# csiro-robotics/syropod_highlevel_controller

Hardware: AMD Instinct MI355X
Metric: control-cycles/sec (all legs IK-solved) (higher is better)
Workload: dtype f64

## Files before the change

### syropod_highlevel_controller_amd/csrc/shc_cycle_kernel.hpp

```cpp
#pragma once

#include "shc_cycle.hpp"
#include "shc_cycle_launch.hpp"

#include <hip/hip_runtime.h>

namespace shc {

#ifndef SHC_WAVES_PER_SIMD
#define SHC_WAVES_PER_SIMD 2
#endif
#ifndef SHC_ROT_WAVES_PER_SIMD
#define SHC_ROT_WAVES_PER_SIMD 1
#endif
#ifndef SHC_TERRAIN_WAVES_PER_SIMD
#define SHC_TERRAIN_WAVES_PER_SIMD 2
#endif

struct LegPlanes {
  double2 *base;
  int64_t ns;
  uint32_t slot;
  typedef double v2d __attribute__((ext_vector_type(2)));
  __device__ __forceinline__ double2 load(int plane) const { return (base + plane * ns)[slot]; }
// ... 343 lines not shown
    if (A.batch_mask & (1u << RG_IMU)) {
      const double *q = bound_array(A, 0, BND_IMUQ) + r * A.kstride[BND_IMUQ], *w = bound_array(A, 0, BND_IMUW) + r * A.kstride[BND_IMUW];
#pragma unroll
      for (int h = 0; h < NI; ++h) {
        const int idx = lane + 64 * h, field = idx / RPW, rr = idx - field * RPW;
        const int64_t rob = rob0 + rr;
        if (field < 7 && rob < st.n_robots) rob_imu[h] = field < 3 ? w[rob * 3 + field] : q[rob * 4 + (field - 3)];
      }
    }
  };
  const auto batch_rob_commit = [&]() {
    if (A.batch_mask & (1u << RG_VEL)) {
      const int field = lane / RPW, rr = lane - field * RPW;
      if (lane < 3 * RPW && wave * RPW + rr < st.n_robots) tile[(R::VIN + field) * RPW + rr] = rob_vel;
    }
    if (A.batch_mask & (1u << RG_IMU)) {
#pragma unroll
      for (int h = 0; h < NI; ++h) {
        const int idx = lane + 64 * h, field = idx / RPW, rr = idx - field * RPW;
        if (field < 7 && wave * RPW + rr < st.n_robots) tile[(R::GYRO + field) * RPW + rr] = rob_imu[h];
      }
      __builtin_amdgcn_fence(__ATOMIC_RELEASE, "wavefront");
      __builtin_amdgcn_wave_barrier();
      if (lane < RPW && wave * RPW + lane < st.n_robots) {
        const Quat qn = normalized(Quat{tile[(R::IMUQ + 0) * RPW + lane], tile[(R::IMUQ + 1) * RPW + lane], tile[(R::IMUQ + 2) * RPW + lane], tile[(R::IMUQ + 3) * RPW + lane]});
        tile[(R::IMUQ + 0) * RPW + lane] = qn.w, tile[(R::IMUQ + 1) * RPW + lane] = qn.x, tile[(R::IMUQ + 2) * RPW + lane] = qn.y, tile[(R::IMUQ + 3) * RPW + lane] = qn.z;
      }
    }
    __builtin_amdgcn_fence(__ATOMIC_RELEASE, "wavefront");
    __builtin_amdgcn_wave_barrier();
  };
  if constexpr (batch) batch_rob_issue(0);
  for (;;) {
    unsigned db = unsigned(gate), sp = unsigned(gate >> 32);
    if constexpr (batch) {
      if (c >= sp) break;
      h0 = u64(c) + 1, h1 = u64(A.batch_mask) | kResidentDirect;
      hdr_valid = true;
    }
    if (!batch && !(c < db && c < sp)) {
      if (c >= sp) break;
      asm volatile("s_waitcnt vmcnt(0)" ::: "memory");
      if (lane == 0) st_agent(A.progress + wave, u64(c));
      const u64 t0 = wall_clock64();
      for (;;) {
        __builtin_amdgcn_s_sleep(4);
        gate = uni64(ld_agent(&A.ctl->gate));
        db = unsigned(gate), sp = unsigned(gate >> 32);
        if (c >= sp || c < db) break;
        if (wall_clock64() - t0 > emergency_ticks) {
          held.fault = true;
          break;
        }
      }
      if (held.fault || c >= sp) break;
      hdr_valid = false;
    }
    if (!hdr_valid) {
      const u64 *hp = reinterpret_cast<const u64 *>(A.headers + (c & (kResidentHeaders - 1)));
      h0 = uni64(ld_agent(hp));
      h1 = uni64(ld_agent(hp + 1));
    }
    u64 gate_next_v = gate;
    if constexpr (!batch) gate_next_v = ld_agent(&A.ctl->gate);
    const bool next_valid = !batch && db > c + 1;
    u64 n0v = 0, n1v = 0;
    if (next_valid) {
      const u64 *hp = reinterpret_cast<const u64 *>(A.headers + ((c + 1) & (kResidentHeaders - 1)));
      n0v = ld_agent(hp);
      n1v = ld_agent(hp + 1);
    }
    const int64_t row = batch ? int64_t(c) : 0;
    if constexpr (batch) {
      held.seen |= A.batch_mask;
      if (A.batch_mask & (1u << RG_FORCE)) held.src_force = -2;
      if (A.batch_mask & (1u << RG_EFFORT)) held.src_effort = -2;
      batch_rob_commit();
      if (c + 1 < A.batch_cycles) batch_rob_issue(int64_t(c) + 1);
    } else {
      resident_take_inputs<64 / L, ROBOT_ALL, true>(A, c, h0, h1, wave, lane, tile, tile_i, dirty, held, st.n_robots, row);
    }
// ... 68 lines not shown
    const V3 f = in.force();
    planes[(FD::FORCE_IN / 2) * ns + slot] = double2{f.x, f.y};
    planes[(FD::FORCE_IN / 2 + 1) * ns + slot] = double2{f.z, 0.0};
  }
  if (held.src_effort != -1) {
    double ef[NJ];
    in.effort(ef);
#pragma unroll
    for (int p = 0; p < FD::NJE / 2; ++p) planes[(FD::EFFORT_IN / 2 + p) * ns + slot] = double2{ef[2 * p], 2 * p + 1 < NJ ? ef[2 * p + 1] : 0.0};
  }
}

template <int L, int NJ, unsigned F>
__device__ __forceinline__ void resident_epilogue(const ResidentArgs &A, const DevState &st, const uint32_t slot, const int lane, const bool live,
                                                  const double *tile, const int32_t *tile_i, double *gtile, int32_t *gtile_i, const ResidentHeld &held) {
  using R = RobotFields;
  using FD = Fields<NJ>;
  constexpr int RPW = 64 / L;
  const int64_t ns = st.n_slots;
  store_rob_fields<RPW, R::VIN, R::CORE_END>(tile, gtile, lane);
  if (held.seen & (1u << RG_IMU)) {
    store_rob_fields<RPW, R::GYRO, R::IMU_END>(tile, gtile, lane);
    store_rob_fields<RPW, R::IMUQ, R::IMUQ_END>(tile, gtile, lane);
  }
  if ((held.seen & (1u << RG_RESET)) && lane < RPW) gtile_i[R::I_RESET_MODE * RPW + lane] = tile_i[R::I_RESET_MODE * RPW + lane];
  if (live) carry_leg_inputs<L, NJ>(A, st, held, ns, slot, int(slot % 64) % L);
  if (lane == 0 && A.batch_cycles == 0) {
    if (held.fault) __hip_atomic_fetch_or(&A.ctl->fault, 1ull, __ATOMIC_RELAXED, __HIP_MEMORY_SCOPE_AGENT);
    __hip_atomic_fetch_add(&A.ctl->exited, 1ull, __ATOMIC_RELAXED, __HIP_MEMORY_SCOPE_AGENT);
  }
}

enum : int { PART_BOTH = 0, PART_GATE = 1, PART_DONE = 2 };
template <int PART>
__device__ __forceinline__ void resident_relay(const ResidentArgs &A) {
  const int lane = threadIdx.x & 63;
  const unsigned max_cycles = A.max_cycles;
  unsigned db = 0, sp = max_cycles, idle_stop = 0xffffffffu;
  u64 reason = RESIDENT_EXIT_MAX, last_reason = 0, last_gate = ~0ull, last_done = 0, iter = 0;
  u64 t_last = wall_clock64(), t_all_done = 0;
  for (;;) {
    const u64 now = wall_clock64();
    const u64 exited_v = ld_agent(&A.ctl->exited);
    const u64 gate_v = PART == PART_DONE ? ld_agent(&A.ctl->gate) : 0;
    const u64 done_v = PART != PART_DONE ? ld_agent(&A.ctl->pad[1]) : 0;
    u64 pv[8];
    if (PART != PART_GATE) {
#pragma unroll
      for (int j = 0; j < 8; ++j) pv[j] = j * 64 + lane < A.n_waves ? ld_agent(A.progress + j * 64 + lane) : ~0ull;
    }
    if (PART != PART_DONE) {
      const u64 hd_v = ld_sys(&A.host->doorbell), hs_v = ld_sys(&A.host->stop);
      const u64 rec_v = lane < 2 ? ld_sys(&A.host->records[size_t(db & (kResidentHeaders - 1)) * 2 + lane]) : 0;
      const u64 hd = uni64(hd_v), hs = uni64(hs_v);
      unsigned want_db = hd > max_cycles ? max_cycles : unsigned(hd);
      if (want_db < db) want_db = db;
      if (want_db == db && db < max_cycles) {
        const u64 tag = u64(db) + 1;
        const bool word_ok = lane == 0 ? rec_v == tag : (lane == 1 ? (rec_v >> 48) == (tag & 0xffffull) : true);
        if (__all(word_ok)) {
          const u64 w1 = uni64(__shfl(rec_v, 1, 64));
          if (lane == 0) {
            u64 *hp = reinterpret_cast<u64 *>(A.headers + (db & (kResidentHeaders - 1)));
            st_agent(hp + 1, (w1 & 0x7fffull) | u64(kResidentDirect) | (w1 & 0x30000ull));
            st_agent(hp, tag);
          }
          asm volatile("s_waitcnt vmcnt(0)" ::: "memory");
          want_db = db + 1;
        }
      }
      if (want_db != db || uni64(done_v) < u64(db)) t_last = now;
      else if (idle_stop == 0xffffffffu && now - t_last > A.idle_ticks) idle_stop = db;
      unsigned want_sp = max_cycles;
      u64 why = RESIDENT_EXIT_MAX;
      if (hs <= max_cycles) want_sp = unsigned(hs), why = RESIDENT_EXIT_STOP;
      if (idle_stop < want_sp) want_sp = idle_stop, why = RESIDENT_EXIT_IDLE;
      if (want_sp < db) want_sp = db;
      if (want_db > want_sp) want_db = want_sp;
      db = want_db, sp = want_sp, reason = why;
      if (reason != last_reason) {
        if (lane == 0) st_agent(&A.ctl->pad[0], reason);
        last_reason = reason;
      }
      const u64 gate = (u64(sp) << 32) | db;
      if (gate != last_gate) {
        if (lane == 0) st_agent(&A.ctl->gate, gate);
        last_gate = gate;
      }
    }
    const u64 exited = uni64(exited_v);
    bool leave = exited == u64(A.n_waves);
    if (PART != PART_GATE) {
      if (PART == PART_DONE) sp = unsigned(uni64(gate_v) >> 32);
      u64 m = ~0ull;
#pragma unroll
      for (int j = 0; j < 8; ++j) m = pv[j] < m ? pv[j] : m;
      for (int64_t base = 512; base < A.n_waves; base += 512) {
        u64 v[8];
#pragma unroll
        for (int j = 0; j < 8; ++j) {
          const int64_t w = base + j * 64 + lane;
          v[j] = w < A.n_waves ? ld_agent(A.progress + w) : ~0ull;
        }
#pragma unroll
        for (int j = 0; j < 8; ++j) m = v[j] < m ? v[j] : m;
      }
#pragma unroll
      for (int off = 32; off > 0; off >>= 1) {
        const u64 o = __shfl_xor(m, off, 64);
        m = o < m ? o : m;
      }
      m = uni64(m);
      if (m != last_done) {
        if (lane == 0) {
          st_sys(&A.host->done, m);
          st_agent(&A.ctl->pad[1], m);
        }
        last_done = m;
      }
      bool gave_up = false;
      if (!leave && m >= sp) {
        if (t_all_done == 0) t_all_done = now;
        else if (now - t_all_done > 5000 * A.ticks_per_ms) leave = gave_up = true;
      }
      if (leave) {
        const u64 fault = uni64(ld_agent(&A.ctl->fault));
        const u64 why = uni64(ld_agent(&A.ctl->pad[0]));
        if (lane == 0) {
          st_sys(&A.host->fault, fault);
          st_sys(&A.host->done, m);
          st_agent(&A.ctl->pad[1], m);
          asm volatile("s_waitcnt vmcnt(0)" ::: "memory");
          st_agent(&A.ctl->pad[2], 1ull);
          st_sys(&A.host->exited, (fault || gave_up) ? u64(RESIDENT_EXIT_FAULT) : why);
        }
      }
      if ((++iter & 1023) == 0 && lane == 0) st_sys(&A.host->heartbeat, iter);
    }
    if (leave) break;
    __builtin_amdgcn_s_sleep(1);
  }
}

template <int L, int NJ, unsigned F, bool RES, int HALF = ROLE_ALL, bool BATCH = false>
__device__ __forceinline__ void cycle_wave(const DevState &st, const SharedConsts<L, NJ> *gc, int n_cycles, unsigned rt_flags, const int64_t wave,
                                           const ResidentArgs *ra) {
  static_assert(HALF == ROLE_ALL || (!RES && (F & (F_DYN | F_TERRAIN | F_MLEGS | F_AUTO)) == 0), "half-step launches: feature-exact kernels without auto posing / terrain paths");
  using R = RobotFields;
  using FT = Feat<F>;
  constexpr int RPW = 64 / L;
  __shared__ SharedConsts<L, NJ> C;
  extern __shared__ double wave_lds[];
  constexpr int kWaveDoubles = R::COUNT * RPW + PK_COUNT * 64 + (R::I_COUNT * RPW + 1) / 2;
  SHC_TICK(0);
  const bool manual_live = (rt_flags & RT_MANUAL_LIVE) != 0;
  const bool touchdown_detection = (rt_flags & RT_TOUCHDOWN) != 0;
  const int lane = threadIdx.x & 63;
  const int wib = threadIdx.x >> 6;
  const int64_t rob0 = wave * RPW;
  const int64_t left = st.n_robots - rob0;
  const int robots_here = left < RPW ? (left < 0 ? 0 : int(left)) : RPW;
  int grp = lane / L;
  const int leg = lane - grp * L;
  const bool live = grp < robots_here;
  if (grp >= robots_here) grp = robots_here > 0 ? robots_here - 1 : 0;
// ... 430 lines not shown
#ifdef SHC_ABLATE
        if (!(P.debug_skip & 65536))
#endif
        if (POSE_SPLIT) publish_for_pose(c_front + 1, fb.plane_prev_changed);
        SHC_TICK(29);
        double *mb = &X.mailbox[pair][c_front & 1][0][lane];
        mb[0] = out.poser_tip.x, mb[64] = out.poser_tip.y, mb[128] = out.poser_tip.z;
        if constexpr (ODOM_WALKER) {
          if (FT::odom(P) && __any(fb.odom_run)) {
            if (fb.odom_run) {
              if constexpr (ODOM_REGS) odometry_advance(odom[0], odom[1], odom[2], odom[3], P, fb.odom_vel.x, fb.odom_vel.y, fb.odom_vel.z, &odom_cache);
              else odometry_step(rb, P, fb.odom_vel.x, fb.odom_vel.y, fb.odom_vel.z, &odom_cache);
            }
          }
        } else if (FT::odom(P)) {
          mb[192] = fb.odom_vel.x, mb[256] = fb.odom_vel.y, mb[320] = fb.odom_vel.z, mb[384] = fb.odom_run ? 1.0 : 0.0;
        }
        SHC_TICK(22);
      }
      SHC_TICK(23);
      if (kind == IT_EXIT) break;
      SHC_R2_ITER_END(0, 19, 20, 21, 2, 3, 4, 5, 6, 7, 16, 8, 17, 15, 29, 22, 23);
      if (kind == IT_REAL) ++c_front;
      prev_real = kind == IT_REAL;
      __syncthreads();
      ++k;
    }
  } else {
    for (;;) {
      SHC_R2_ITER_BEGIN();
      const int kind = __builtin_amdgcn_readfirstlane(int(X.ctrl[k & 3][0]));
      const u64 h0 = uni64(X.ctrl[k & 3][1]), h1 = uni64(X.ctrl[k & 3][2]);
      SHC_TICK(29);
      int nk = IT_EXIT;
      u64 nh0v = 0, nh1v = 0;
      if (leader && kind != IT_EXIT) {
        u64 gate;
        if (kind == IT_BUBBLE) {
          __builtin_amdgcn_s_sleep(2);
          gate = uni64(ld_agent(&A.ctl->gate));
        } else {
          gate = uni64(gate_pref);
        }
        const unsigned db = unsigned(gate), sp = unsigned(gate >> 32);
        const unsigned cn = c_front + (kind == IT_REAL ? 1u : 0u);
        nk = cn >= sp ? IT_EXIT : (cn < db ? IT_REAL : IT_BUBBLE);
        if (nk == IT_BUBBLE) {
          const u64 now = wall_clock64();
          if (bubble_since == 0) bubble_since = now;
          else if (now - bubble_since > emergency_ticks) nk = IT_EXIT, held.fault = true;
        } else {
          bubble_since = 0;
        }
        if (nk == IT_REAL) {
          const u64 *hp = reinterpret_cast<const u64 *>(A.headers + (cn & (kResidentHeaders - 1)));
          nh0v = ld_agent(hp);
          nh1v = ld_agent(hp + 1);
        }
        if (kind == IT_BUBBLE) gate_pref = gate;
        else gate_pref = ld_agent(&A.ctl->gate);
      }
      if (active) {
        SHC_TICK(24);
        if constexpr (POSE_SPLIT) if (kind == IT_REAL) {
          resident_take_inputs<RPW, ROBOT_POSE, false>(A, c_front, h0, h1, wave, lane, tile, tile_i, dirty, held, st.n_robots);
          SHC_TICK(30);
          double pose_c = -1.0;
#pragma unroll
          for (int j = 0; j < L; ++j) {
            const double cj = X.pose_c[pair][c_front & 1][g.base + j];
            pose_c = cj >= 0.0 ? cj : pose_c;
          }
          int lw[L] = {};
          const double *mb = &X.mailbox[pair][c_front & 1][0][lane];
          const V3 plane_prev{mb[7 * 64], mb[8 * 64], mb[9 * 64]}, pnorm_prev{mb[10 * 64], mb[11 * 64], mb[12 * 64]};
          int rword_unused = 0;
          Pose ap = pose_identity(), la = pose_identity();
#ifdef SHC_ABLATE
          if (!(P.debug_skip & 2048))
#endif
          (void)cycle_pose<L, NJ, F, true>(s, C, P, C.leg[leg], rb, g, leg, lw, rword_unused, 0, dirty, manual_live, ap, la, plane_prev, pnorm_prev, fb.uf.swing_c_count, 0,
                                           &owpp_cache, &pose_c);
          __builtin_amdgcn_fence(__ATOMIC_RELEASE, "workgroup");
          __builtin_amdgcn_wave_barrier();
          if (lane == 0) *const_cast<volatile unsigned *>(&X.pose_done[pair]) = c_front + 1;
        }
        SHC_TICK(25);
        if (prev_real) {
          resident_take_inputs<RPW, ROBOT_NONE, true>(A, c_back, prev_h0, prev_h1, wave, lane, tile, tile_i, dirty, held, st.n_robots);
          if (held.src_force != in_src_force || held.src_effort != in_src_effort) {
            in_at = leg_inputs_in_force<L, NJ>(A, st.legd, held.src_force, held.src_effort, ns, slot, wave * RPW + grp, leg);
            in_src_force = held.src_force, in_src_effort = held.src_effort;
          }
          LegInRing<NJ> in = in_at;
          if (FT::tipf(P)) in.prefetch_effort();
          SHC_TICK(31);
// ... 8 lines not shown
              }
            }
          }
          out.adm_delta = V3{0, 0, 0};
          if (FT::adm(P)) cycle_admittance<NJ>(s, out, P, in);
          s.word = 0;
          SHC_TICK(26);
          cycle_back<L, NJ, F>(s, out, C, leg, st.legd, ns, slot, nullptr, in, fb);
          SHC_TICK(27);
          asm volatile("s_waitcnt vmcnt(0)" ::: "memory");
          if (lane == 0) st_agent(A.progress + wave, u64(c_back));
          SHC_TICK(13);
          {
            typedef unsigned v4u __attribute__((ext_vector_type(4)));
            double flat[2 * NJ];
#pragma unroll
            for (int i = 0; i < NJ; ++i) flat[FD::Q + i] = s.q[i], flat[FD::QD + i] = s.qd[i];
            const unsigned soff = oslot * out_slot_bytes;
#ifdef SHC_ABLATE
            if (!(P.debug_skip & 4096))
#endif
            if (live) {
#pragma unroll
              for (int p = 0; p < NJ; ++p) {
                const u64 a = u64(__double_as_longlong(flat[2 * p])), b = u64(__double_as_longlong(flat[2 * p + 1]));
                const v4u w = {unsigned(a), unsigned(a >> 32), unsigned(b), unsigned(b >> 32)};
                __builtin_amdgcn_raw_buffer_store_b128(w, out_rsrc, unsigned((int64_t(p) * ns + slot) * 16), soff, 16 );
              }
            }
          }
          ++c_back;
          oslot = oslot + 1 == unsigned(A.depth) ? 0 : oslot + 1;
          SHC_TICK(28);
        }
        if (kind != IT_REAL) {
          asm volatile("s_waitcnt vmcnt(0)" ::: "memory");
          if (lane == 0) st_agent(A.progress + wave, u64(c_back));
        }
      }
      if (leader && kind != IT_EXIT && lane == 0) {
        X.ctrl[(k + 1) & 3][0] = u64(nk);
        X.ctrl[(k + 1) & 3][1] = nh0v;
        X.ctrl[(k + 1) & 3][2] = nh1v;
      }
      SHC_TICK(14);
      if (kind == IT_EXIT) break;
      SHC_R2_ITER_END(128, 19, 29, 24, 30, 25, 31, 26, 9, 10, 11, 12, 27, 13, 28, 14);
      if (kind == IT_REAL) ++c_front;
      prev_real = kind == IT_REAL;
      prev_h0 = h0, prev_h1 = h1;
      __syncthreads();
      ++k;
    }
  }
#undef SHC_R2_ITER_BEGIN
#undef SHC_R2_ITER_END
#undef SHC_R2_PHASES
#ifdef SHC_RES2_TIMING
  if (blockIdx.x == 1 && lane == 0 && pair == 0) {
    unsigned long long *dbg = reinterpret_cast<unsigned long long *>(A.ctl) + 8 + (walker ? 0 : 4);
    dbg[0] = tm_busy, dbg[1] = tm_real, dbg[2] = __builtin_readcyclecounter() - tm_total0, dbg[3] = k;
#ifndef SHC_RES2_BUSY_ONLY
    if (walker) {
      for (int i = 0; i < 32; ++i) dbg[8 + i] = (unsigned long long)shc_acc_lds[i];
    } else {
      for (int i = 0; i < 32; ++i) dbg[36 + i] = (unsigned long long)shc_acc_lds[32 + i];
    }
#endif
  }
#endif
  if (active && ODOM_REGS && FT::odom(P) && walker == ODOM_WALKER) {
#pragma unroll
    for (int i = 0; i < 4; ++i) rb.put(R::ODOM + i, odom[i]);
  }
  if (active) {
    if (walker) {
      X.stiff[pair][lane] = s.stiff;
// ... 56 lines not shown
```

### syropod_highlevel_controller_amd/csrc/shc_cycle_launch.hpp

```cpp
#pragma once

#include "shc_cycle.hpp"

#include <hip/hip_runtime.h>

namespace shc {

enum : int { RG_VEL = 0, RG_IMU = 1, RG_POSE = 2, RG_RESET = 3, RG_FORCE = 4, RG_EFFORT = 5, RG_COUNT = 6 };
enum : int { RIN_VEL = 0, RIN_IMU = 3, RIN_POSE = 10, RIN_COUNT = 16 };

constexpr int kResidentHeaders = 1024;
constexpr int kBoundSets = 4;
enum : int { BND_LIN = 0, BND_ANG = 1, BND_IMUQ = 2, BND_IMUW = 3, BND_FORCE = 4, BND_EFFORT = 5, BND_COUNT = 6 };
constexpr unsigned kResidentDirect = 1u << 15;
struct ResidentCtl {
  unsigned long long gate;
  unsigned long long exited;
  unsigned long long fault;
  unsigned long long pad[5];
  unsigned long long dbg[80];
};
struct ResidentHost {
  unsigned long long doorbell;
  unsigned long long stop;
  unsigned long long done;
  unsigned long long exited;
  unsigned long long heartbeat;
  unsigned long long fault;
  unsigned long long late_reads;
  unsigned long long pad_[1];
  unsigned long long records[kResidentHeaders * 2];
};
struct ResidentHeader {
  unsigned long long tag;
  unsigned short mask;
  unsigned char pos[RG_COUNT];
};
static_assert(sizeof(ResidentHeader) == 16, "header is read as two 8-byte words");
enum : unsigned long long { RESIDENT_EXIT_STOP = 1, RESIDENT_EXIT_IDLE = 2, RESIDENT_EXIT_MAX = 3, RESIDENT_EXIT_FAULT = 4 };

struct ResidentArgs {
  ResidentCtl *ctl;
  ResidentHost *host;
  unsigned long long *progress;
  ResidentHeader *headers;
  const double *bound[kBoundSets][BND_COUNT];
  const double *rin;
  const int32_t *rini;
  const double *force;
  const double *effort;
  double *out;
  int depth;
  unsigned max_cycles;
  unsigned long long idle_ticks;
  unsigned long long ticks_per_ms;
  int64_t n_waves;
  double touchdown_threshold, liftoff_threshold;
  unsigned batch_cycles, batch_mask;
  int64_t kstride[BND_COUNT];
  int64_t batch_wave0;
};

struct ResidentFit;
struct CycleLaunch {
  DevState st;
  const void *consts;
  const CycleParams *cp;
  unsigned rt_flags;
  bool generic;
  hipStream_t stream;
  unsigned grid;
// ... 21 lines not shown
```

### syropod_highlevel_controller_amd/csrc/shc_resident.hpp

```cpp

struct Resident {
  bool active = false;
  int depth = 0;
  ResidentArgs args{};
  ResidentHost *host = nullptr;
  ResidentHost *host_dev = nullptr;
  ResidentCtl *ctl = nullptr;
  unsigned long long *progress = nullptr;
  ResidentHeader *headers = nullptr;
  double *rin = nullptr, *force = nullptr, *effort = nullptr, *out = nullptr, *stage = nullptr;
  int32_t *rini = nullptr;
  size_t stage_bytes = 0;
  static constexpr int kPinSlots = 4;
  unsigned *post_blocks_done = nullptr;
  char *pin = nullptr, *pin_dev = nullptr;
  hipEvent_t pin_ev[kPinSlots] = {};
  unsigned long long pin_uses = 0;
  hipStream_t in_stream = nullptr;
  hipStream_t loop_stream = nullptr;
  hipEvent_t loop_ev = nullptr;
  unsigned long long published = 0;
  unsigned long long posted = 0;
  unsigned long long posts[RG_COUNT] = {};
  std::vector<unsigned long long> post_cycle[RG_COUNT];
  unsigned max_cycles = 0;
  unsigned long long wall_khz = 100000;
  bool poisoned = false;
  bool stream_doorbell_pending = false;
  unsigned groups_posted = 0;
  bool two_wave = false;
  long long direct_last = -1;
};

__global__ void resident_doorbell_kernel(ResidentHost *host, unsigned long long value) {
  __hip_atomic_store(&host->doorbell, value, __ATOMIC_RELAXED, __HIP_MEMORY_SCOPE_SYSTEM);
}

struct ResidentPost {
  const double *lin, *ang, *imu_q, *imu_w, *tvi, *rvi, *force, *effort;
  const int32_t *reset;
  int pos[RG_COUNT];
  unsigned mask;
  unsigned long long cycle;
  unsigned long long doorbell;
  ResidentHost *host;
  unsigned *blocks_done;
};
__global__ void resident_post_kernel(ResidentPost pp, ResidentArgs A, ResidentHeader *headers, double *rin, int32_t *rini, double *force, double *effort,
                                     int64_t n, int L, int NJ, int64_t n_slots) {
  const int64_t t = int64_t(blockIdx.x) * blockDim.x + threadIdx.x;
  const int rpw = 64 / L;
  auto put = [](double *p, double v) {
    __hip_atomic_store(reinterpret_cast<unsigned long long *>(p), (unsigned long long)__double_as_longlong(v), __ATOMIC_RELAXED, __HIP_MEMORY_SCOPE_AGENT);
  };
// ... 194 lines not shown
    if ((err = hipEventCreateWithFlags(&r->loop_ev, hipEventDisableTiming)) != hipSuccess) return bail(err, "hipEventCreate");
    r->stage_bytes = size_t(e->n) * (16 * 8 + 8) + size_t(e->n) * e->L * (3 + e->NJ) * 8 + 256;
    const size_t D = size_t(ring_depth);
    if ((err = hipMalloc(&r->ctl, sizeof(ResidentCtl))) != hipSuccess) return bail(err, "hipMalloc");
    if ((err = hipMalloc(&r->progress, size_t(e->n_waves) * 8)) != hipSuccess) return bail(err, "hipMalloc");
    if ((err = hipMalloc(&r->headers, sizeof(ResidentHeader) * kResidentHeaders)) != hipSuccess) return bail(err, "hipMalloc");
    if ((err = hipMalloc(&r->rin, D * e->n_waves * RIN_COUNT * rpw * 8)) != hipSuccess) return bail(err, "hipMalloc");
    if ((err = hipMalloc(&r->rini, D * e->n_waves * rpw * 8)) != hipSuccess) return bail(err, "hipMalloc");
    if ((err = hipMalloc(&r->force, D * 2 * e->n_slots * 16)) != hipSuccess) return bail(err, "hipMalloc");
    if ((err = hipMalloc(&r->effort, D * (NJE / 2) * e->n_slots * 16)) != hipSuccess) return bail(err, "hipMalloc");
    if ((err = hipMalloc(&r->out, D * out_slot_bytes)) != hipSuccess) return bail(err, "hipMalloc");
    if ((err = hipMalloc(&r->stage, r->stage_bytes)) != hipSuccess) return bail(err, "hipMalloc");
    if ((err = hipMalloc(&r->post_blocks_done, 64)) != hipSuccess) return bail(err, "hipMalloc");
    if ((err = hipMemsetAsync(r->post_blocks_done, 0, 64, e->stream)) != hipSuccess) return bail(err, "hipMemset");
    if ((err = hipHostMalloc(reinterpret_cast<void **>(&r->pin), r->stage_bytes * Resident::kPinSlots, hipHostMallocMapped)) != hipSuccess)
      return bail(err, "hipHostMalloc(input staging)");
    if ((err = hipHostGetDevicePointer(reinterpret_cast<void **>(&r->pin_dev), r->pin, 0)) != hipSuccess) return bail(err, "hipHostGetDevicePointer");
    for (hipEvent_t &ev : r->pin_ev)
      if ((err = hipEventCreateWithFlags(&ev, hipEventDisableTiming)) != hipSuccess) return bail(err, "hipEventCreate");
    for (int gi = 0; gi < RG_COUNT; ++gi) r->post_cycle[gi].assign(D, 0);
  }
  Resident *r = e->res;
  {
    ResidentCtl ctl0{};
    ctl0.gate = (unsigned long long)(unsigned(max_cycles)) << 32;
    HIP_TRY(hipMemcpyAsync(r->ctl, &ctl0, sizeof ctl0, hipMemcpyHostToDevice, e->stream));
    HIP_TRY(hipStreamSynchronize(e->stream));
  }
  HIP_TRY(hipMemsetAsync(r->progress, 0, size_t(e->n_waves) * 8, e->stream));
  HIP_TRY(hipMemsetAsync(r->headers, 0, sizeof(ResidentHeader) * kResidentHeaders, e->stream));
  memset(r->host, 0, sizeof(ResidentHost));
  r->host->stop = ~0ull;
  __sync_synchronize();
  r->published = r->posted = 0;
  r->direct_last = -1;
  r->groups_posted = 0;
  r->stream_doorbell_pending = false;
  for (int gi = 0; gi < RG_COUNT; ++gi) {
    r->posts[gi] = 0;
    std::fill(r->post_cycle[gi].begin(), r->post_cycle[gi].end(), 0ull);
  }
  r->max_cycles = unsigned(max_cycles);
  ResidentArgs &A = r->args;
  A.ctl = r->ctl;
  A.host = r->host_dev;
  A.progress = r->progress;
  A.headers = r->headers;
  memcpy(A.bound, e->bound_inputs, sizeof A.bound);
  A.rin = r->rin;
  A.rini = r->rini;
  A.force = r->force;
  A.effort = r->effort;
  A.out = r->out;
  A.depth = ring_depth;
  A.max_cycles = r->max_cycles;
  int wall_khz = 0;
  if (hipDeviceGetAttribute(&wall_khz, hipDeviceAttributeWallClockRate, e->device) != hipSuccess || wall_khz <= 0) wall_khz = 100000;
  r->wall_khz = (unsigned long long)wall_khz;
  A.idle_ticks = (unsigned long long)(idle_timeout_ms ? idle_timeout_ms : 5000) * r->wall_khz;
  A.ticks_per_ms = r->wall_khz;
  A.n_waves = e->n_waves;
  A.touchdown_threshold = e->params.touchdown_threshold;
  A.liftoff_threshold = e->params.liftoff_threshold;
  e->plan_poser_tips_current = false;
  const bool two_wave = fit.two_wave && !(e->features & SHC_FEAT_RESIDENT_ONE_WAVE) && (e->n_waves + 1) / 2 + 1 <= prop.multiProcessorCount;
  r->two_wave = two_wave;
  HIP_TRY(hipEventRecord(r->loop_ev, e->stream));
// ... 43 lines not shown
  if (in->pose_translation_velocity) mask |= 1u << RG_POSE;
  if (in->pose_reset_mode) mask |= 1u << RG_RESET;
  if (in->tip_force) mask |= 1u << RG_FORCE;
  if (in->joint_effort) mask |= 1u << RG_EFFORT;
  if ((mask & ((1u << RG_POSE) | (1u << RG_RESET))) && !(e->rt_flags & RT_MANUAL_LIVE))
    return fail(SHC_ERR_UNSUPPORTED, "pose inputs: give the engine one (shc_engine_set_pose_input / set_pose_reset_mode) before shc_engine_resident_begin");
  if ((mask & (1u << RG_EFFORT)) && !(e->rt_flags & RT_EFFORT_LIVE))
    return fail(SHC_ERR_UNSUPPORTED, "joint efforts: give the engine one (shc_engine_set_joint_effort) before shc_engine_resident_begin");
  const unsigned long long c = r->posted;
  if (c < r->published) return fail(SHC_ERR_INVALID_ARG, "resident mode: this cycle has already been published without inputs");
  if (c >= r->max_cycles) return fail(SHC_ERR_INVALID_ARG, "resident mode: past max_cycles");
  HIP_TRY(hipSetDevice(e->device));
  const double patience = 5.0;
  if (c >= kResidentHeaders && !spin_until([&] { return host_load(&r->host->done) > c - kResidentHeaders; }, patience))
    return fail(SHC_ERR_TIMEOUT, "resident mode: 1024 posted cycles are waiting to run");
  if (in->direct) {
    const int set = in->direct - 1;
    if (set < 0 || set >= kBoundSets) return fail(SHC_ERR_INVALID_ARG, "direct: bound input set 1 .. 4");
    if (mask & ((1u << RG_POSE) | (1u << RG_RESET))) return fail(SHC_ERR_INVALID_ARG, "direct posts carry velocity, IMU, tip force and joint effort; post pose inputs / reset modes the ordinary way");
    if (mask == 0) return fail(SHC_ERR_INVALID_ARG, "direct post without inputs (use shc_engine_resident_publish)");
    const int need[RG_COUNT] = {BND_LIN, BND_IMUQ, -1, -1, BND_FORCE, BND_EFFORT};
    for (int gi = 0; gi < RG_COUNT; ++gi)
      if ((mask & (1u << gi)) && (need[gi] < 0 || !r->args.bound[set][need[gi]]))
        return fail(SHC_ERR_INVALID_ARG, "direct post: that group is not part of the bound input set (shc_engine_resident_bind_inputs before shc_engine_resident_begin)");
    if (r->published < c) {
      const int rc2 = shc_engine_resident_publish(e, int64_t(c - r->published));
      if (rc2 != SHC_OK) return rc2;
    }
    const unsigned long long tag = c + 1;
    volatile unsigned long long *rec = r->host->records + size_t(c & (kResidentHeaders - 1)) * 2;
    rec[1] = (unsigned long long)mask | ((unsigned long long)set << 16) | ((tag & 0xffffull) << 48);
    host_store(const_cast<unsigned long long *>(&rec[0]), tag);
    r->groups_posted |= mask;
    r->posted = r->published = c + 1;
    r->direct_last = (long long)c;
    if (cycle) *cycle = int64_t(c);
    return SHC_OK;
  }
  ResidentPost pp{};
  pp.mask = mask;
  pp.cycle = c;
  for (int gi = 0; gi < RG_COUNT; ++gi) {
    if (!(mask & (1u << gi))) continue;
    const unsigned long long k = r->posts[gi];
    pp.pos[gi] = int(k % r->depth);
    if (k >= (unsigned long long)r->depth) {
      const unsigned long long successor_cycle = r->post_cycle[gi][(k + 1) % r->depth];
      if (!spin_until([&] { return host_load(&r->host->done) >= successor_cycle || host_load(&r->host->exited) != 0; }, patience))
        return fail(SHC_ERR_TIMEOUT, "resident mode: ring_depth posted input sets are waiting to be consumed (publish them)");
    }
  }
  size_t off = 0;
  const int pin_slot = int(r->pin_uses % Resident::kPinSlots);
  if (!in->on_device && r->pin_uses >= (unsigned long long)Resident::kPinSlots) HIP_TRY(hipEventSynchronize(r->pin_ev[pin_slot]));
  auto dev = [&](const void *src, size_t bytes, const void **out) -> int {
    if (in->on_device) {
      *out = src;
      return SHC_OK;
    }
    if (off + bytes > r->stage_bytes) return fail(SHC_ERR_INVALID_ARG, "staging buffer too small");
    const size_t at = size_t(pin_slot) * r->stage_bytes + off;
    memcpy(r->pin + at, src, bytes);
    *out = r->pin_dev + at;
    off += (bytes + 15) & ~size_t(15);
    return SHC_OK;
  };
  const size_t n = size_t(e->n), nl = n * e->L;
#define STAGE(field, member, bytes)                                                              \
  if (in->member) {                                                                              \
    const void *d_;                                                                              \
    if ((rc = dev(in->member, bytes, &d_)) != SHC_OK) return rc;                                 \
    pp.field = reinterpret_cast<decltype(pp.field)>(d_);                                         \
  }
  STAGE(lin, linear_xy, n * 16)
  STAGE(ang, angular, n * 8)
  STAGE(imu_q, imu_orientation_wxyz, n * 32)
  STAGE(imu_w, imu_angular_velocity, n * 24)
  STAGE(tvi, pose_translation_velocity, n * 24)
  STAGE(rvi, pose_rotation_velocity, n * 24)
  STAGE(reset, pose_reset_mode, n * 4)
  STAGE(force, tip_force, nl * 24)
  STAGE(effort, joint_effort, nl * e->NJ * 8)
#undef STAGE
  const int64_t threads = (mask & ((1u << RG_FORCE) | (1u << RG_EFFORT))) ? int64_t(nl) : int64_t(n);
  const bool publish = in->publish != 0;
  if (publish) {
    if ((rc = resident_wait_direct_installed(r)) != SHC_OK) return rc;
    pp.doorbell = c + 1;
    pp.host = r->host_dev;
    pp.blocks_done = r->post_blocks_done;
  }
  resident_post_kernel<<<dim3((unsigned)((threads + 63) / 64)), dim3(64), 0, r->in_stream>>>(pp, r->args, r->headers, r->rin, r->rini, r->force, r->effort,
                                                                                              e->n, e->L, e->NJ, e->n_slots);
  HIP_TRY(hipGetLastError());
  if (!in->on_device) {
    HIP_TRY(hipEventRecord(r->pin_ev[pin_slot], r->in_stream));
    r->pin_uses++;
  }
  for (int gi = 0; gi < RG_COUNT; ++gi)
    if (mask & (1u << gi)) {
      r->post_cycle[gi][r->posts[gi] % r->depth] = c;
      r->posts[gi]++;
    }
  r->groups_posted |= mask;
  r->posted = c + 1;
  if (publish) r->published = c + 1;
  r->stream_doorbell_pending = true;
  if (cycle) *cycle = int64_t(c);
  return SHC_OK;
}

extern "C" int shc_engine_resident_publish(shc_engine *e, int64_t n_cycles) {
  int rc = resident_require(e, true);
  if (rc != SHC_OK) return rc;
  Resident *r = e->res;
  if ((rc = resident_alive(r)) != SHC_OK) return rc;
  if (n_cycles < 0) return fail(SHC_ERR_INVALID_ARG, "n_cycles < 0");
  if (n_cycles == 0) return SHC_OK;
  if (r->published + (unsigned long long)n_cycles > r->max_cycles) return fail(SHC_ERR_INVALID_ARG, "resident mode: past max_cycles");
  if ((rc = resident_wait_direct_installed(r)) != SHC_OK) return rc;
  r->published += (unsigned long long)n_cycles;
  if (r->posted < r->published) r->posted = r->published;
  if (r->stream_doorbell_pending) {
    HIP_TRY(hipSetDevice(e->device));
    if (hipStreamQuery(r->in_stream) == hipSuccess) {
      r->stream_doorbell_pending = false;
    } else {
      resident_doorbell_kernel<<<dim3(1), dim3(1), 0, r->in_stream>>>(r->host_dev, r->published);
      HIP_TRY(hipGetLastError());
      return SHC_OK;
    }
  }
  host_store(&r->host->doorbell, r->published);
  return SHC_OK;
}

extern "C" int shc_engine_resident_wait(shc_engine *e, int64_t cycles, int timeout_ms) {
  int rc = resident_require(e, true);
  if (rc != SHC_OK) return rc;
  Resident *r = e->res;
  if (cycles < 0 || (unsigned long long)cycles > r->published) return fail(SHC_ERR_INVALID_ARG, "resident mode: waiting for cycles that were not published");
  const unsigned long long want = (unsigned long long)cycles;
  if (!spin_until([&] { return host_load(&r->host->done) >= want || host_load(&r->host->exited) != 0; }, timeout_ms > 0 ? timeout_ms * 1e-3 : 10.0))
    return fail(SHC_ERR_TIMEOUT, "resident mode: the published cycles did not complete in time");
  if (host_load(&r->host->done) < want) return fail(SHC_ERR_TIMEOUT, "resident mode: the device loop stopped before these cycles ran");
  return SHC_OK;
}

extern "C" int shc_engine_resident_get_joint_state(shc_engine *e, int64_t cycle, double *q, double *qd, int on_device) {
  int rc = resident_require(e, true);
  if (rc != SHC_OK) return rc;
  Resident *r = e->res;
  const unsigned long long done = host_load(&r->host->done);
  if (cycle < 0 || (unsigned long long)cycle >= done) return fail(SHC_ERR_INVALID_ARG, "resident mode: that cycle has not completed (shc_engine_resident_wait)");
  if (r->published > (unsigned long long)cycle + r->depth)
    return fail(SHC_ERR_INVALID_ARG, "resident mode: that cycle's outputs may have been overwritten (ring_depth newer cycles were published)");
  HIP_TRY(hipSetDevice(e->device));
  const double *slot = r->out + size_t(cycle % r->depth) * size_t(e->NJ) * e->n_slots * 2;
  const int64_t threads = e->n * e->L;
  for (int which = 0; which < 2; ++which) {
    double *dst = which ? qd : q;
    if (!dst) continue;
    double *d = on_device ? dst : r->stage;
    gather_leg_kernel<<<dim3((unsigned)((threads + 63) / 64)), dim3(64), 0, r->in_stream>>>(d, slot, e->n_slots, e->n, e->L, e->NJ,
                                                                                            which ? LEG_FIELD(e, QD) : LEG_FIELD(e, Q));
    HIP_TRY(hipGetLastError());
// ... 31 lines not shown
  resident_wait_done_kernel<<<dim3(1), dim3(1), 0, e->stream>>>(r->ctl, r->host_dev, (unsigned long long)cycle + 1, ticks);
  HIP_TRY(hipGetLastError());
  const double *slot = r->out + size_t(cycle % r->depth) * size_t(e->NJ) * e->n_slots * 2;
  const int64_t threads = e->n * e->L;
  for (int which = 0; which < 2; ++which) {
    double *dst = which ? qd : q;
    if (!dst) continue;
    gather_leg_kernel<<<dim3((unsigned)((threads + 63) / 64)), dim3(64), 0, e->stream>>>(dst, slot, e->n_slots, e->n, e->L, e->NJ,
                                                                                         which ? LEG_FIELD(e, QD) : LEG_FIELD(e, Q));
    HIP_TRY(hipGetLastError());
  }
  return SHC_OK;
}

extern "C" int shc_engine_resident_status(shc_engine *e, int64_t *published, int64_t *completed, int32_t *running) {
  int rc = resident_require(e, false);
  if (rc != SHC_OK) return rc;
  Resident *r = e->res;
  const bool active = r && r->active;
  if (published) *published = active ? int64_t(r->published) : 0;
  if (completed) *completed = active ? int64_t(host_load(&r->host->done)) : 0;
  if (running) *running = active && host_load(&r->host->exited) == 0 ? 1 : 0;
  return SHC_OK;
}

extern "C" int shc_engine_resident_end(shc_engine *e, int64_t *cycles_run) {
  int rc = resident_require(e, true);
  if (rc != SHC_OK) return rc;
  Resident *r = e->res;
  HIP_TRY(hipSetDevice(e->device));
  HIP_TRY(hipStreamSynchronize(r->in_stream));
  const int direct_rc = resident_wait_direct_installed(r);
  const std::string direct_msg = direct_rc != SHC_OK ? std::string(shc_last_error()) : std::string();
  if (direct_rc == SHC_OK) host_store(&r->host->doorbell, r->published);
  host_store(&r->host->stop, direct_rc == SHC_OK ? r->published : 0ull);
  const bool answered = spin_until([&] { return host_load(&r->host->exited) != 0; }, r->poisoned ? 5.0 : 30.0);
  if (!answered) {
    r->poisoned = true;
    return fail(SHC_ERR_TIMEOUT, "resident mode: the device loop did not answer the stop request in time; the engine stays in resident mode - call "
                                 "shc_engine_resident_end again");
  }
  hipError_t err = hipStreamSynchronize(r->loop_stream);
  if (err == hipSuccess) err = hipStreamSynchronize(e->stream);
  r->active = false;
  r->poisoned = false;
#ifdef SHC_RES2_TIMING
  if (err == hipSuccess) {
    ResidentCtl c;
    (void)hipMemcpy(&c, r->ctl, sizeof c, hipMemcpyDeviceToHost);
    for (int w = 0; w < 2; ++w)
      fprintf(stderr, "[res2 timing] %s: %.0f clocks busy per steady REAL iteration (%llu of them), loop %llu clocks, %llu iterations\n", w ? "model " : "walker",
              c.dbg[4 * w + 1] ? double(c.dbg[4 * w]) / double(c.dbg[4 * w + 1]) : 0.0, c.dbg[4 * w + 1], c.dbg[4 * w + 2], c.dbg[4 * w + 3]);
#ifndef SHC_RES2_BUSY_ONLY
    const int order[] = {20, 21, 2, 3, 4, 5, 6, 7, 16, 8, 17, 15, 29, 22, 23};
    const char *wname[] = {"control words (LDS) read", "inputs of the cycle taken", "cycle_front entry", "robot word / command read, stop predicates", "(pose elsewhere)", "getLimit",
                           "velocity shaping", "walk state machine", "stepper (stride, Bezier, tip)", "tip rotation / iteratePhase / planes / leg word", "wait for the pose flag",
                           "pose read + updateStance", "control input for the next pose published", "mailbox written", "to the barrier"};
    const double its = c.dbg[1] ? double(c.dbg[1]) : 1.0;
    fprintf(stderr, "[res2 timing] walker of pair 0, mean clocks per phase:\n");
    for (int i = 0; i < int(sizeof(order) / sizeof(int)); ++i) fprintf(stderr, "[res2 timing]   walker t%-2d %-58s %7.0f\n", order[i], wname[i], double(c.dbg[8 + order[i]]) / its);
    const int morder[] = {29, 24, 30, 25, 31, 26, 9, 10, 11, 12, 27, 13, 28, 14};
    const char *mname[] = {"control words (LDS) read", "leader: gate, what the next iteration is, header prefetch issued", "pose inputs of the cycle taken",
                           "updateCurrentPose of the walker's cycle + flag", "leg inputs in force, joint efforts prefetched", "mailbox read, odometry, admittance",
                           "cycle_back entry (desired tip)", "IK step + joint update", "sin / cos, chain, Jacobian", "model tip, tip force", "cycle_back exit",
                           "wait for the previous stores + progress word", "output-ring stores issued", "control words written (leader: waits for its loads)"};
    const double mits = c.dbg[5] ? double(c.dbg[5]) : 1.0;
    fprintf(stderr, "[res2 timing] model wavefront of pair 0 (the leader), mean clocks per phase:\n");
    for (int i = 0; i < int(sizeof(morder) / sizeof(int)); ++i) fprintf(stderr, "[res2 timing]   model  t%-2d %-58s %7.0f\n", morder[i], mname[i], double(c.dbg[40 + morder[i]]) / mits);
#endif
  }
#endif
  const unsigned long long reason = host_load(&r->host->exited), done = host_load(&r->host->done);
  if (cycles_run) *cycles_run = int64_t(done);
  if (r->groups_posted & (1u << RG_FORCE)) e->rt_flags |= RT_TOUCHDOWN;
  if (err != hipSuccess) return fail(SHC_ERR_HIP, std::string("hipStreamSynchronize: ") + hipGetErrorString(err));
  if (direct_rc != SHC_OK) return fail(direct_rc, direct_msg + " (the loop was stopped after " + std::to_string(done) + " cycles)");
  if (reason == RESIDENT_EXIT_FAULT || host_load(&r->host->fault) != 0)
    return fail(SHC_ERR_HIP, "resident mode: a wavefront gave up waiting for the relay; restore the engine from a snapshot");
  if (host_load(&r->host->late_reads) != 0)
    return fail(SHC_ERR_TIMEOUT, "resident mode: a stream-ordered read (shc_engine_resident_get_joint_state_async) gave up waiting for its cycle");
  if (!((reason == RESIDENT_EXIT_STOP || reason == RESIDENT_EXIT_MAX) && done == r->published))
    return fail(SHC_ERR_TIMEOUT, std::string("resident mode: the device loop had stopped by itself (") +
                                     (reason == RESIDENT_EXIT_IDLE ? "idle timeout" : reason == RESIDENT_EXIT_MAX ? "max_cycles" : "unknown") + ") after " +
                                     std::to_string(done) + " of " + std::to_string(r->published) + " published cycles");
  return SHC_OK;
}

static int step_k_out_ring(shc_engine *e, int K) {
  const size_t need = size_t(K) * size_t(e->NJ) * size_t(e->n_slots) * 16;
  if (e->k_out && e->k_out_bytes >= need) return SHC_OK;
  if (e->k_out) {
    const int rc = join_side(e);
    if (rc != SHC_OK) return rc;
    HIP_TRY(hipStreamSynchronize(e->stream));
    (void)hipFree(e->k_out);
    e->k_out = nullptr, e->k_out_bytes = 0;
  }
  HIP_TRY(hipMalloc(reinterpret_cast<void **>(&e->k_out), need));
  e->k_out_bytes = need;
  return SHC_OK;
}

// ... 132 lines not shown
```

Before: 1.579 billion.

## Add bare-gate flag to skip header reload and trim bubble-iteration sync

The doorbell word now carries the header-end cycle in its upper 32 bits. The relay uses it to set a 'bare' bit in the gate when a release carries no new header, and the leader then skips the header loads on bubble-to-real transitions. The leader's bubble path is restructured so the gate poll overlaps the model half, the sleep only happens after consecutive bubbles, and the progress store runs only on the first bubble after a real cycle. Optional hop-timing instrumentation is added behind a macro. The aim is to cut release latency for single-tick bursts, at the cost of more complex gate encoding and a risk of using stale headers if the bare bit is wrong.

Result: no change. 1.571 billion (-0.5%).

```diff
diff --git a/syropod_highlevel_controller_amd/csrc/shc_cycle_kernel.hpp b/syropod_highlevel_controller_amd/csrc/shc_cycle_kernel.hpp
--- a/syropod_highlevel_controller_amd/csrc/shc_cycle_kernel.hpp
+++ b/syropod_highlevel_controller_amd/csrc/shc_cycle_kernel.hpp
@@ -399,7 +399,7 @@
   };
   if constexpr (batch) batch_rob_issue(0);
   for (;;) {
-    unsigned db = unsigned(gate), sp = unsigned(gate >> 32);
+    unsigned db = unsigned(gate) & kGateCycles, sp = unsigned(gate >> 32);
     if constexpr (batch) {
       if (c >= sp) break;
       h0 = u64(c) + 1, h1 = u64(A.batch_mask) | kResidentDirect;
@@ -413,7 +413,7 @@
       for (;;) {
         __builtin_amdgcn_s_sleep(4);
         gate = uni64(ld_agent(&A.ctl->gate));
-        db = unsigned(gate), sp = unsigned(gate >> 32);
+        db = unsigned(gate) & kGateCycles, sp = unsigned(gate >> 32);
         if (c >= sp || c < db) break;
         if (wall_clock64() - t0 > emergency_ticks) {
           held.fault = true;
@@ -548,13 +548,22 @@
 }
 
 enum : int { PART_BOTH = 0, PART_GATE = 1, PART_DONE = 2 };
+#ifdef SHC_RES2_HOPS
+#define SHC_HOP(i, cond) do { if ((cond) && lane == 0) st_agent(&A.ctl->dbg[8 + (i)], wall_clock64()); } while (0)
+#else
+#define SHC_HOP(i, cond) do {} while (0)
+#endif
 template <int PART>
 __device__ __forceinline__ void resident_relay(const ResidentArgs &A) {
   const int lane = threadIdx.x & 63;
   const unsigned max_cycles = A.max_cycles;
   unsigned db = 0, sp = max_cycles, idle_stop = 0xffffffffu;
+  bool bare = false;
   u64 reason = RESIDENT_EXIT_MAX, last_reason = 0, last_gate = ~0ull, last_done = 0, iter = 0;
   u64 t_last = wall_clock64(), t_all_done = 0;
+#ifdef SHC_RES2_HOPS
+  u64 hop_sum = 0, hop_n = 0;
+#endif
   for (;;) {
     const u64 now = wall_clock64();
     const u64 exited_v = ld_agent(&A.ctl->exited);
@@ -568,9 +577,11 @@
     if (PART != PART_DONE) {
       const u64 hd_v = ld_sys(&A.host->doorbell), hs_v = ld_sys(&A.host->stop);
       const u64 rec_v = lane < 2 ? ld_sys(&A.host->records[size_t(db & (kResidentHeaders - 1)) * 2 + lane]) : 0;
-      const u64 hd = uni64(hd_v), hs = uni64(hs_v);
+      const u64 hdw = uni64(hd_v), hs = uni64(hs_v);
+      const u64 hd = hdw & 0xffffffffull, hdr_end = hdw >> 32;
       unsigned want_db = hd > max_cycles ? max_cycles : unsigned(hd);
       if (want_db < db) want_db = db;
+      bool want_bare = hdr_end <= u64(db) && uni64(done_v) == u64(db);
       if (want_db == db && db < max_cycles) {
         const u64 tag = u64(db) + 1;
         const bool word_ok = lane == 0 ? rec_v == tag : (lane == 1 ? (rec_v >> 48) == (tag & 0xffffull) : true);
@@ -583,6 +594,7 @@
           }
           asm volatile("s_waitcnt vmcnt(0)" ::: "memory");
           want_db = db + 1;
+          want_bare = false;
         }
       }
       if (want_db != db || uni64(done_v) < u64(db)) t_last = now;
@@ -593,14 +605,19 @@
       if (idle_stop < want_sp) want_sp = idle_stop, why = RESIDENT_EXIT_IDLE;
       if (want_sp < db) want_sp = db;
       if (want_db > want_sp) want_db = want_sp;
+      if (want_db != db) bare = want_bare;
       db = want_db, sp = want_sp, reason = why;
       if (reason != last_reason) {
         if (lane == 0) st_agent(&A.ctl->pad[0], reason);
         last_reason = reason;
       }
-      const u64 gate = (u64(sp) << 32) | db;
+      const u64 gate = (u64(sp) << 32) | db | (bare ? u64(kGateBare) : 0);
       if (gate != last_gate) {
         if (lane == 0) st_agent(&A.ctl->gate, gate);
+#ifdef SHC_RES2_HOPS
+        if (lane == 0 && ((gate ^ last_gate) & kGateCycles)) st_agent(&A.ctl->dbg[8 + HOP_POLL], now);
+        SHC_HOP(HOP_GATE, ((gate ^ last_gate) & kGateCycles) != 0);
+#endif
         last_gate = gate;
       }
     }
@@ -632,6 +649,14 @@
           st_sys(&A.host->done, m);
           st_agent(&A.ctl->pad[1], m);
         }
+#ifdef SHC_RES2_HOPS
+        if (m == last_done + 1) {
+          const u64 t_host = wall_clock64();
+          const u64 sv = lane < HOP_SWEEP ? ld_agent(&A.ctl->dbg[8 + lane]) : (lane == HOP_SWEEP ? now : t_host);
+          const u64 d = sv - uni64(__shfl(sv, HOP_POLL, 64));
+          if (__all(lane >= HOP_COUNT || d < 100000)) hop_sum += d, ++hop_n;
+        }
+#endif
         last_done = m;
       }
       bool gave_up = false;
@@ -640,6 +665,10 @@
         else if (now - t_all_done > 5000 * A.ticks_per_ms) leave = gave_up = true;
       }
       if (leave) {
+#ifdef SHC_RES2_HOPS
+        if (lane < HOP_COUNT) st_agent(&A.ctl->dbg[24 + lane], hop_sum);
+        asm volatile("s_waitcnt vmcnt(0)" ::: "memory");
+#endif
         const u64 fault = uni64(ld_agent(&A.ctl->fault));
         const u64 why = uni64(ld_agent(&A.ctl->pad[0]));
         if (lane == 0) {
@@ -647,6 +676,9 @@
           st_sys(&A.host->done, m);
           st_agent(&A.ctl->pad[1], m);
           asm volatile("s_waitcnt vmcnt(0)" ::: "memory");
+#ifdef SHC_RES2_HOPS
+          st_agent(&A.ctl->dbg[23], hop_n);
+#endif
           st_agent(&A.ctl->pad[2], 1ull);
           st_sys(&A.host->exited, (fault || gave_up) ? u64(RESIDENT_EXIT_FAULT) : why);
         }
@@ -1143,17 +1175,12 @@
       const int kind = __builtin_amdgcn_readfirstlane(int(X.ctrl[k & 3][0]));
       const u64 h0 = uni64(X.ctrl[k & 3][1]), h1 = uni64(X.ctrl[k & 3][2]);
       SHC_TICK(29);
+      SHC_HOP(HOP_FRONT, blockIdx.x == 1 && leader && kind == IT_REAL && !prev_real);
+      SHC_HOP(HOP_DRAIN_ITER, blockIdx.x == 1 && leader && kind != IT_REAL && prev_real);
       int nk = IT_EXIT;
       u64 nh0v = 0, nh1v = 0;
-      if (leader && kind != IT_EXIT) {
-        u64 gate;
-        if (kind == IT_BUBBLE) {
-          __builtin_amdgcn_s_sleep(2);
-          gate = uni64(ld_agent(&A.ctl->gate));
-        } else {
-          gate = uni64(gate_pref);
-        }
-        const unsigned db = unsigned(gate), sp = unsigned(gate >> 32);
+      const auto decide = [&](const u64 gate) {
+        const unsigned db = unsigned(gate) & kGateCycles, sp = unsigned(gate >> 32);
         const unsigned cn = c_front + (kind == IT_REAL ? 1u : 0u);
         nk = cn >= sp ? IT_EXIT : (cn < db ? IT_REAL : IT_BUBBLE);
         if (nk == IT_BUBBLE) {
@@ -1163,16 +1190,24 @@
         } else {
           bubble_since = 0;
         }
-        if (nk == IT_REAL) {
+        SHC_HOP(HOP_SEEN, blockIdx.x == 1 && kind == IT_BUBBLE && nk == IT_REAL);
+        if (nk == IT_REAL && !(kind == IT_BUBBLE && (gate & kGateBare))) {
           const u64 *hp = reinterpret_cast<const u64 *>(A.headers + (cn & (kResidentHeaders - 1)));
           nh0v = ld_agent(hp);
           nh1v = ld_agent(hp + 1);
         }
-        if (kind == IT_BUBBLE) gate_pref = gate;
-        else gate_pref = ld_agent(&A.ctl->gate);
+      };
+      u64 gate_now = 0;
+      if (leader && kind == IT_REAL) {
+        decide(uni64(gate_pref));
+        gate_pref = ld_agent(&A.ctl->gate);
+      } else if (leader && kind == IT_BUBBLE) {
+        if (!prev_real) __builtin_amdgcn_s_sleep(2);
+        gate_now = ld_agent(&A.ctl->gate);
       }
       if (active) {
         SHC_TICK(24);
+        SHC_HOP(HOP_BACK, blockIdx.x == 1 && leader && kind != IT_REAL && prev_real);
         if constexpr (POSE_SPLIT) if (kind == IT_REAL) {
           resident_take_inputs<RPW, ROBOT_POSE, false>(A, c_front, h0, h1, wave, lane, tile, tile_i, dirty, held, st.n_robots);
           SHC_TICK(30);
@@ -1247,17 +1282,29 @@
           ++c_back;
           oslot = oslot + 1 == unsigned(A.depth) ? 0 : oslot + 1;
           SHC_TICK(28);
-        }
-        if (kind != IT_REAL) {
+          SHC_HOP(HOP_STORES, blockIdx.x == 1 && leader && kind != IT_REAL);
+        }
+        if (kind != IT_REAL && prev_real) {
           asm volatile("s_waitcnt vmcnt(0)" ::: "memory");
           if (lane == 0) st_agent(A.progress + wave, u64(c_back));
-        }
+          SHC_HOP(HOP_PROGRESS, blockIdx.x == 1 && leader && prev_real);
+        }
+      }
+      if (leader && kind == IT_BUBBLE) {
+        gate_pref = uni64(gate_now);
+        decide(gate_pref);
       }
       if (leader && kind != IT_EXIT && lane == 0) {
         X.ctrl[(k + 1) & 3][0] = u64(nk);
         X.ctrl[(k + 1) & 3][1] = nh0v;
         X.ctrl[(k + 1) & 3][2] = nh1v;
       }
+#ifdef SHC_RES2_HOPS
+      if (blockIdx.x == 1 && leader && kind == IT_BUBBLE && nk == IT_REAL) {
+        asm volatile("s_waitcnt vmcnt(0) lgkmcnt(0)" ::: "memory");
+        SHC_HOP(HOP_HEADER, true);
+      }
+#endif
       SHC_TICK(14);
       if (kind == IT_EXIT) break;
       SHC_R2_ITER_END(128, 19, 29, 24, 30, 25, 31, 26, 9, 10, 11, 12, 27, 13, 28, 14);
diff --git a/syropod_highlevel_controller_amd/csrc/shc_cycle_launch.hpp b/syropod_highlevel_controller_amd/csrc/shc_cycle_launch.hpp
--- a/syropod_highlevel_controller_amd/csrc/shc_cycle_launch.hpp
+++ b/syropod_highlevel_controller_amd/csrc/shc_cycle_launch.hpp
@@ -13,6 +13,7 @@
 constexpr int kBoundSets = 4;
 enum : int { BND_LIN = 0, BND_ANG = 1, BND_IMUQ = 2, BND_IMUW = 3, BND_FORCE = 4, BND_EFFORT = 5, BND_COUNT = 6 };
 constexpr unsigned kResidentDirect = 1u << 15;
+constexpr unsigned kGateCycles = 0x7fffffffu, kGateBare = 0x80000000u;
 struct ResidentCtl {
   unsigned long long gate;
   unsigned long long exited;
@@ -37,6 +38,7 @@
   unsigned char pos[RG_COUNT];
 };
 static_assert(sizeof(ResidentHeader) == 16, "header is read as two 8-byte words");
+enum : int { HOP_POLL = 0, HOP_GATE, HOP_SEEN, HOP_HEADER, HOP_FRONT, HOP_DRAIN_ITER, HOP_BACK, HOP_STORES, HOP_PROGRESS, HOP_SWEEP, HOP_HOST, HOP_COUNT };
 enum : unsigned long long { RESIDENT_EXIT_STOP = 1, RESIDENT_EXIT_IDLE = 2, RESIDENT_EXIT_MAX = 3, RESIDENT_EXIT_FAULT = 4 };
 
 struct ResidentArgs {
diff --git a/syropod_highlevel_controller_amd/csrc/shc_resident.hpp b/syropod_highlevel_controller_amd/csrc/shc_resident.hpp
--- a/syropod_highlevel_controller_amd/csrc/shc_resident.hpp
+++ b/syropod_highlevel_controller_amd/csrc/shc_resident.hpp
@@ -20,6 +20,8 @@
   hipStream_t loop_stream = nullptr;
   hipEvent_t loop_ev = nullptr;
   unsigned long long published = 0;
+  unsigned long long hdr_end = 0;
+  unsigned long long doorbell_word() const { return published | (hdr_end << 32); }
   unsigned long long posted = 0;
   unsigned long long posts[RG_COUNT] = {};
   std::vector<unsigned long long> post_cycle[RG_COUNT];
@@ -280,7 +282,7 @@
   memset(r->host, 0, sizeof(ResidentHost));
   r->host->stop = ~0ull;
   __sync_synchronize();
-  r->published = r->posted = 0;
+  r->published = r->posted = r->hdr_end = 0;
   r->direct_last = -1;
   r->groups_posted = 0;
   r->stream_doorbell_pending = false;
@@ -390,7 +392,7 @@
     rec[1] = (unsigned long long)mask | ((unsigned long long)set << 16) | ((tag & 0xffffull) << 48);
     host_store(const_cast<unsigned long long *>(&rec[0]), tag);
     r->groups_posted |= mask;
-    r->posted = r->published = c + 1;
+    r->posted = r->published = r->hdr_end = c + 1;
     r->direct_last = (long long)c;
     if (cycle) *cycle = int64_t(c);
     return SHC_OK;
@@ -444,7 +446,7 @@
   const bool publish = in->publish != 0;
   if (publish) {
     if ((rc = resident_wait_direct_installed(r)) != SHC_OK) return rc;
-    pp.doorbell = c + 1;
+    pp.doorbell = (c + 1) | ((c + 1) << 32);
     pp.host = r->host_dev;
     pp.blocks_done = r->post_blocks_done;
   }
@@ -461,7 +463,7 @@
       r->posts[gi]++;
     }
   r->groups_posted |= mask;
-  r->posted = c + 1;
+  r->posted = r->hdr_end = c + 1;
   if (publish) r->published = c + 1;
   r->stream_doorbell_pending = true;
   if (cycle) *cycle = int64_t(c);
@@ -484,12 +486,12 @@
     if (hipStreamQuery(r->in_stream) == hipSuccess) {
       r->stream_doorbell_pending = false;
     } else {
-      resident_doorbell_kernel<<<dim3(1), dim3(1), 0, r->in_stream>>>(r->host_dev, r->published);
+      resident_doorbell_kernel<<<dim3(1), dim3(1), 0, r->in_stream>>>(r->host_dev, r->doorbell_word());
       HIP_TRY(hipGetLastError());
       return SHC_OK;
     }
   }
-  host_store(&r->host->doorbell, r->published);
+  host_store(&r->host->doorbell, r->doorbell_word());
   return SHC_OK;
 }
 
@@ -587,7 +589,7 @@
   HIP_TRY(hipStreamSynchronize(r->in_stream));
   const int direct_rc = resident_wait_direct_installed(r);
   const std::string direct_msg = direct_rc != SHC_OK ? std::string(shc_last_error()) : std::string();
-  if (direct_rc == SHC_OK) host_store(&r->host->doorbell, r->published);
+  if (direct_rc == SHC_OK) host_store(&r->host->doorbell, r->doorbell_word());
   host_store(&r->host->stop, direct_rc == SHC_OK ? r->published : 0ull);
   const bool answered = spin_until([&] { return host_load(&r->host->exited) != 0; }, r->poisoned ? 5.0 : 30.0);
   if (!answered) {
@@ -623,6 +625,21 @@
     fprintf(stderr, "[res2 timing] model wavefront of pair 0 (the leader), mean clocks per phase:\n");
     for (int i = 0; i < int(sizeof(morder) / sizeof(int)); ++i) fprintf(stderr, "[res2 timing]   model  t%-2d %-58s %7.0f\n", morder[i], mname[i], double(c.dbg[40 + morder[i]]) / mits);
 #endif
+#ifdef SHC_RES2_HOPS
+    if (c.dbg[23]) {
+      const char *hname[HOP_COUNT] = {"relay: the poll that saw the doorbell is issued (PCIe read)", "relay: gate stored", "leader: release seen in a bubble iteration",
+                                      "leader: header in hand, control words written", "first REAL iteration begins (walker half)", "next iteration begins (model half, pipeline drains)",
+                                      "leader: through its gate poll, model half begins", "output-ring stores issued", "stores drained, progress word written",
+                                      "relay: the sweep that saw every progress word is issued", "relay: done stored to the host"};
+      fprintf(stderr, "[res2 hops] one-tick bursts: %llu, mean microseconds since the relay's poll (and since the previous hop)\n", c.dbg[23]);
+      double prev = 0.0;
+      for (int i = 0; i < HOP_COUNT; ++i) {
+        const double us = double(c.dbg[24 + i]) / double(c.dbg[23]) * 1e3 / double(r->wall_khz);
+        fprintf(stderr, "[res2 hops]   %-2d %-64s %7.2f  (+%5.2f)\n", i, hname[i], us, us - prev);
+        prev = us;
+      }
+    }
+#endif
   }
 #endif
   const unsigned long long reason = host_load(&r->host->exited), done = host_load(&r->host->done);
```
